# qq456cvb/CanonicalVoting

Measured on AMD Instinct MI355X. Metric: scenes/sec (80k-pt synthetic scans), higher is better.
Workload: dtype f32

## Files before the change

### canonicalvoting_amd/csrc/cv_common.h

```cpp
#pragma once
#include <hip/hip_runtime.h>

#include <cstdarg>
#include <cstdint>
#include <cstdio>

#include "cv_hip.h"

void cv_set_error(const char* fmt, ...);

#define CV_HIP_CHECK(expr)                                                                  \
    do {                                                                                    \
        hipError_t e_ = (expr);                                                             \
        if (e_ != hipSuccess) {                                                             \
            cv_set_error("%s failed: %s (%s:%d)", #expr, hipGetErrorString(e_), __FILE__,   \
                         __LINE__);                                                         \
            return CV_EHIP;                                                                 \
        }                                                                                   \
    } while (0)

#define CV_LAUNCH_CHECK() CV_HIP_CHECK(hipGetLastError())

#define CV_REQUIRE(cond, code, ...)     \
    do {                                \
        if (!(cond)) {                  \
            cv_set_error(__VA_ARGS__);  \
            return (code);              \
        }                               \
    } while (0)

__host__ __device__ static inline size_t cv_align_up(size_t v, size_t a) { return (v + a - 1) / a * a; }

struct CvCarver {
    char* base;
    size_t off = 0;
    explicit CvCarver(void* p) : base(static_cast<char*>(p)) {}
    template <typename T>
    T* take(size_t count) {
        off = cv_align_up(off, 256);
        T* r = reinterpret_cast<T*>(base + off);
        off += count * sizeof(T);
        return r;
    }
};

struct CvMapJob {
    const int32_t* out_coords; long long n_out;
    const unsigned long long* keys; const int32_t* vals; long long cap;
    int k, ts;
    int32_t* nbr;
    const int32_t* compose;
    const unsigned* bitmap;
    const int32_t* bbox;
    int up;
};
constexpr int CV_MAX_MAP_JOBS = 12;
int cv_sp_kernel_maps_batch(const CvMapJob* jobs, int n_jobs, void* stream);
constexpr long long CV_BITMAP_WORDS = 1ll << 20;
int cv_sp_occupancy_bitmap(const int32_t* d_coords, long long n, const int32_t* d_bbox, unsigned* d_bits, void* stream,
                           bool pre_cleared = false);

int cv_sp_build_levels_zero(int32_t* const* d_coords, unsigned long long* const* d_keys, int32_t* const* d_vals,
                            long long n, long long cap, int num_levels, int32_t* d_counts, int32_t* h_counts, void* d_ws,
                            size_t ws_bytes, int32_t* d_zero, long long n_zero, int32_t* d_set_one, void* stream,
                            uint32_t* d_bits = nullptr);

struct CvUpJob { const int32_t* nbr_down; long long n_coarse; int32_t* up; };
int cv_sp_up_maps_batch(const CvUpJob* jobs, int n_jobs, void* stream);

struct CvPermJob { const int32_t* nbr; long long n; int K, groups; int32_t* perm; int with_map; };
constexpr int CV_MAX_PERM_JOBS = 8;
int cv_hv_minmax_async_ex(const float* d_points, int64_t n, float* h_minmax6, void* d_ws, size_t ws_bytes, int32_t* d_zero_word,
                          int32_t* d_fill7f, void* stream);
int cv_decode_f32_ev(float* d_grid_obj, const float* d_grid_rot, const float* d_grid_scale, const int dims[3],
                     const float h_corner3[3], float res, const float* d_points, const float* d_xyz, const float* d_prob,
                     const int32_t* d_class, int64_t n, const cv_decode_params* params, int mutate_grid, void* d_ws, size_t ws_bytes,
                     int* h_n_cand, int64_t* h_cand_idx, int32_t* h_verdict, int* h_n_boxes, float* h_boxes, float* h_scores,
                     int32_t* h_classes, int* h_truncated, void* stream, void* ev_done);
int cv_decode_cat_f32_ev(float* d_grid_obj, const float* d_grid_rot, const float* d_grid_scale, const int dims[3],
                         const float h_corner3[3], float res, const float* d_points, const float* d_xyz, const float* d_prob,
                         const int32_t* d_class, int64_t n, int num_cats, const cv_decode_params* params, int mutate_grid,
                         void* d_ws, size_t ws_bytes, int* h_n_cand, int64_t* h_cand_idx, int32_t* h_verdict, int* h_n_boxes,
                         float* h_boxes, float* h_scores, int32_t* h_classes, int* h_truncated, void* stream, void* ev_done);
int cv_sp_sort_rows_ex(const int32_t* d_coords, long long n, int32_t* d_sorted, int32_t* d_perm, int32_t* d_inv, void* d_ws,
                       size_t ws_bytes, bool single_batch, void* stream, bool bounds_prefilled = false);
int cv_sp_scene_plan_ex(const int32_t* d_input, long long n, int32_t* d_perm, int32_t* d_inv, int32_t* const* d_coords,
                        unsigned long long* const* d_keys, int32_t* const* d_vals, long long cap, int32_t* d_counts,
                        int32_t* h_counts, int stem_k, int mask_groups, long long masked_min_rows,
                        int32_t* d_arena, size_t arena_words, cv_scene_maps* offsets, void* d_sort_ws, size_t sort_ws_bytes,
                        void* d_levels_ws, size_t levels_ws_bytes, bool single_batch, void* stream,
                        bool bounds_prefilled = false);
int cv_sp_mask_perms_batch(const CvPermJob* jobs, int n_jobs, void* d_ws, size_t ws_bytes, void* stream,
                           bool pre_zeroed = false);
```

### canonicalvoting_amd/csrc/net_exec.cpp

```cpp
#include <algorithm>
#include <cstdlib>
#include <mutex>
#include <unordered_map>
#include <vector>

#include "cv_common.h"

namespace {

struct Slot { char* ptr; int ld; long long rows; };

}

extern "C" {

static void scene_maps_layout(const long long* rows, long long n_orig, int stem_k, int mask_groups,
                              long long masked_min_rows, cv_scene_maps* o, size_t* total) {
    size_t off = 0;
    auto take = [&](size_t words) { const size_t at = off; off += cv_align_up(words, 64); return (long long)at; };
    const size_t K5 = (size_t)stem_k * stem_k * stem_k;
    const size_t mp_w = mask_groups > 1 ? (size_t)mask_groups * (1 + (27 + mask_groups - 1) / mask_groups) + (mask_groups + 3) / 4 : 0;
    o->stem = take((size_t)rows[0] * K5);
    o->k3[0] = take((size_t)rows[0] * 27);
    o->mask_perm[0] = (mask_groups > 1 && rows[0] >= masked_min_rows) ? take(mp_w * rows[0]) : -1;
    o->scratch = take((size_t)(5 * std::max(mask_groups, 1) + 4) * 2048);
    o->bitmap = take((size_t)CV_BITMAP_WORDS);
    o->out = -1;
    (void)n_orig;
    for (int i = 0; i < 4; ++i) o->down[i] = take((size_t)rows[i + 1] * 8);
    for (int i = 1; i < 5; ++i) o->k3[i] = take((size_t)rows[i] * 27);
    for (int i = 0; i < 4; ++i) o->up[i] = take((size_t)rows[3 - i] * 8);
    for (int i = 1; i < 5; ++i) o->mask_perm[i] = (mask_groups > 1 && rows[i] >= masked_min_rows) ? take(mp_w * rows[i]) : -1;
    for (int i = 0; i < 4; ++i) o->up_perm[i] = take((size_t)rows[3 - i]);
    *total = off;
}

size_t cv_sp_scene_maps_words(const long long* level_rows, long long n_orig, int stem_k, int mask_groups,
                              long long masked_min_rows, cv_scene_maps* offsets) {
    if (!level_rows || !offsets || n_orig <= 0 || stem_k < 1) return 0;
    size_t total = 0;
    scene_maps_layout(level_rows, n_orig, stem_k, mask_groups, masked_min_rows, offsets, &total);
    return total;
}

static int scene_maps_level0(int32_t* const* d_coords, const unsigned long long* const* d_keys, const int32_t* const* d_vals,
                             long long cap, long long n, const int32_t* d_perm, int stem_k, int mask_groups,
                             const cv_scene_maps& o, int32_t* d_arena, const int32_t* d_bbox, void* stream,
                             bool pre_cleared = false, bool bitmap_filled = false) {
    const unsigned* bits = nullptr;
    if (d_bbox) {
        bits = reinterpret_cast<const unsigned*>(d_arena + o.bitmap);
        if (!bitmap_filled) {
            const int rc0 = cv_sp_occupancy_bitmap(d_coords[0], n, d_bbox, reinterpret_cast<unsigned*>(d_arena + o.bitmap), stream,
                                                   pre_cleared);
            if (rc0 != CV_OK) return rc0;
        }
    }
    CvMapJob mj[2];
    mj[0] = {d_coords[0], n, d_keys[0], d_vals[0], cap, stem_k, 1, d_arena + o.stem, d_perm, bits, d_bbox, 0};
    mj[1] = {d_coords[0], n, d_keys[0], d_vals[0], cap, 3, 1, d_arena + o.k3[0], nullptr, bits, d_bbox, 0};
    int rc = cv_sp_kernel_maps_batch(mj, 2, stream);
    if (rc != CV_OK) return rc;
    if (o.mask_perm[0] >= 0) {
        CvPermJob pj = {d_arena + o.k3[0], n, 27, mask_groups, d_arena + o.mask_perm[0], 1};
        rc = cv_sp_mask_perms_batch(&pj, 1, d_arena + o.scratch, sizeof(int) * (size_t)mask_groups * 2048, stream, pre_cleared);
        if (rc != CV_OK) return rc;
    }
    return CV_OK;
}

static int scene_maps_coarse(int32_t* const* d_coords, const unsigned long long* const* d_keys, const int32_t* const* d_vals,
                             long long cap, const long long* level_rows, int mask_groups, const cv_scene_maps& o,
                             int32_t* d_arena, void* stream, bool pre_zeroed = false) {
    CvMapJob mj[CV_MAX_MAP_JOBS];
    int nm = 0;
    for (int i = 0; i < 4; ++i)
        mj[nm++] = {d_coords[i + 1], level_rows[i + 1], d_keys[i], d_vals[i], cap, 2, 1 << i, d_arena + o.down[i], nullptr, nullptr, nullptr, 0};
    for (int i = 1; i < 5; ++i)
        mj[nm++] = {d_coords[i], level_rows[i], d_keys[i], d_vals[i], cap, 3, 1 << i, d_arena + o.k3[i], nullptr, nullptr, nullptr, 0};
    for (int i = 0; i < 4; ++i) {
        const int fine = 3 - i;
        mj[nm++] = {d_coords[fine], level_rows[fine], d_keys[fine + 1], d_vals[fine + 1], cap, 2, 1 << fine, d_arena + o.up[i],
                    nullptr, nullptr, nullptr, 1};
    }
    int rc = cv_sp_kernel_maps_batch(mj, nm, stream);
    if (rc != CV_OK) return rc;
    CvPermJob pj[CV_MAX_PERM_JOBS];
    int np = 0, groups = 0;
    for (int i = 1; i < 5; ++i)
        if (o.mask_perm[i] >= 0) {
            pj[np++] = {d_arena + o.k3[i], level_rows[i], 27, mask_groups, d_arena + o.mask_perm[i], 1};
            groups += mask_groups;
        }
    for (int i = 0; i < 4; ++i) {
        pj[np++] = {d_arena + o.up[i], level_rows[3 - i], 8, 1, d_arena + o.up_perm[i], 0};
        groups += 1;
    }
    return cv_sp_mask_perms_batch(pj, np, d_arena + o.scratch + (size_t)std::max(mask_groups, 1) * 2048,
                                  sizeof(int) * (size_t)groups * 2048, stream, pre_zeroed);
}

int cv_sp_scene_maps(int32_t* const* d_coords, const unsigned long long* const* d_keys, const int32_t* const* d_vals,
                     long long cap, const long long* level_rows, const int32_t* d_perm, long long n_orig, int stem_k,
                     int mask_groups, long long masked_min_rows, int32_t* d_arena, size_t arena_words, void* stream) {
    CV_REQUIRE(d_coords && d_keys && d_vals && level_rows && d_perm && d_arena, CV_EINVAL, "null pointer argument");
    CV_REQUIRE(n_orig == level_rows[0], CV_EINVAL, "the sorted set must hold the caller's %lld rows", n_orig);
    cv_scene_maps o;
    size_t total = 0;
    scene_maps_layout(level_rows, n_orig, stem_k, mask_groups, masked_min_rows, &o, &total);
    CV_REQUIRE(arena_words >= total, CV_ENOMEM, "scene map arena too small");
    int rc = scene_maps_level0(d_coords, d_keys, d_vals, cap, n_orig, d_perm, stem_k, mask_groups, o, d_arena, nullptr, stream);
    if (rc != CV_OK) return rc;
    return scene_maps_coarse(d_coords, d_keys, d_vals, cap, level_rows, mask_groups, o, d_arena, stream);
}

namespace {
struct PlanSide { hipEvent_t ev; int32_t* h_pinned; int device; };
std::mutex g_plan_mu;
std::unordered_map<int, std::vector<PlanSide>> g_plan_free;
int plan_side_acquire(PlanSide* out) {
    int dev = 0;
    CV_HIP_CHECK(hipGetDevice(&dev));
    {
        std::lock_guard<std::mutex> lk(g_plan_mu);
        auto& pool = g_plan_free[dev];
        if (!pool.empty()) {
            *out = pool.back();
            pool.pop_back();
// ... 178 lines not shown
```

### canonicalvoting_amd/csrc/sparse_conv.hip

```cpp
#include "cv_common.h"

#include <atomic>
#include <cstring>
#include <type_traits>
#include <utility>

#include "sparse_conv_common.h"

using namespace cvsc;

namespace {

template <int NB, bool VEC>
__global__ __launch_bounds__(THREADS) void conv_rows(ConvArgs a) {
    __shared__ float A_s[KC][A_LD];
    __shared__ float B_s[KC][NB * 32];
    __shared__ int nbr_s[TM];
    __shared__ int rows_s[TM];
    __shared__ __attribute__((aligned(16))) float ep_s[4][32][EP_LD];
    const int tid = threadIdx.x, lane = tid & 63, wave = tid >> 6;
    const int n0 = blockIdx.y * (NB * 32);

    if (tid < TM) {
        const long long tile_id = a.row_perm ? (long long)gridDim.x - 1 - blockIdx.x : blockIdx.x;
// ... 1414 lines not shown
        conv_finish_small<<<(unsigned)std::min<long long>((total / 4 + 255) / 256, 16384), 256, 0, st>>>(a);
    else if (a.cout % 4 == 0)
        conv_finish<<<(unsigned)std::min<long long>((total / 4 + 63) / 64, 8192), 256, 0, st>>>(a);
    else
        conv_finish_scalar<<<(unsigned)std::min<long long>((total + 255) / 256, 4096), 256, 0, st>>>(a);
    CV_LAUNCH_CHECK();
    return CV_OK;
}
}
namespace {

__global__ __launch_bounds__(256) void mask_keys(const int* __restrict__ nbr, long long n, int K, int j_begin,
                                                 int j_end, long long* __restrict__ keys) {
    const long long i = blockIdx.x * 256ll + threadIdx.x;
    if (i >= n) return;
    unsigned long long m = 0;
    for (int j = j_begin; j < j_end; ++j)
        if (nbr[i * K + j] >= 0) m |= 1ull << (j - j_begin);
    keys[i] = (long long)m;
}

constexpr int MP_BINS = 1024;
constexpr int MP_THREADS = 1024;

__device__ __forceinline__ int group_mask(const int* __restrict__ nbr, long long row, long long n, int K, int jb, int je) {
    int m = 0;
    for (int j = jb; j < je; ++j)
        if (nbr[row * K + j] >= 0) m |= 1 << (j - jb);
    if (je - jb <= 7) m |= __popc(m) << 7;
    (void)n;
    return m;
}

__global__ __launch_bounds__(MP_THREADS) void mp_hist(const int* __restrict__ nbr, long long n, int K, int groups,
                                                      int* __restrict__ hist ) {
    __shared__ int lh[MP_BINS];
    const int g = blockIdx.y;
    const int jb = K * g / groups, je = K * (g + 1) / groups;
    for (int i = threadIdx.x; i < MP_BINS; i += MP_THREADS) lh[i] = 0;
    __syncthreads();
    const long long row = blockIdx.x * (long long)MP_THREADS + threadIdx.x;
    if (row < n) atomicAdd(&lh[group_mask(nbr, row, n, K, jb, je)], 1);
    __syncthreads();
    for (int i = threadIdx.x; i < MP_BINS; i += MP_THREADS)
        if (lh[i]) atomicAdd(&hist[g * MP_BINS + i], lh[i]);
}

__global__ __launch_bounds__(MP_BINS) void mp_scan(int* __restrict__ hist) {
    __shared__ int s[MP_BINS];
    int* h = hist + blockIdx.x * MP_BINS;
    const int v = h[threadIdx.x];
    s[threadIdx.x] = v;
    __syncthreads();
    for (int off = 1; off < MP_BINS; off <<= 1) {
        const int t = threadIdx.x >= off ? s[threadIdx.x - off] : 0;
        __syncthreads();
        s[threadIdx.x] += t;
        __syncthreads();
    }
    h[threadIdx.x] = s[threadIdx.x] - v;
}

__global__ __launch_bounds__(MP_THREADS) void mp_scatter(const int* __restrict__ nbr, long long n, int K, int groups,
                                                         int* __restrict__ cursor, int* __restrict__ perm,
                                                         int* __restrict__ nbrp, int W) {
    unsigned char* gv = nbrp ? reinterpret_cast<unsigned char*>(nbrp + (long long)groups * n * W) : nullptr;
// ... 14 lines not shown
    __syncthreads();
    if (row < n) {
        const long long pos = (long long)g * n + lh[key] + rank;
        perm[pos] = (int)row;
        if (nbrp) {
            for (int j = jb; j < je; ++j) nbrp[pos * W + (j - jb)] = nbr[row * K + j];
            gv[(long long)g * n + row] = key != 0;
        }
    }
}

struct PermJobsDev {
    CvPermJob j[CV_MAX_PERM_JOBS];
    int group_begin[CV_MAX_PERM_JOBS + 1];
    int n;
};

__device__ __forceinline__ int perm_job_of(const PermJobsDev& jobs, int gy) {
    int ji = 0;
    while (ji + 1 < jobs.n && gy >= jobs.group_begin[ji + 1]) ++ji;
    return ji;
}

__global__ __launch_bounds__(MP_THREADS) void mp_hist_batch(const PermJobsDev jobs, int* __restrict__ hist) {
    __shared__ int lh[MP_BINS];
    const int ji = perm_job_of(jobs, blockIdx.y);
    const CvPermJob& jb = jobs.j[ji];
    const long long row = blockIdx.x * (long long)MP_THREADS + threadIdx.x;
    if (blockIdx.x * (long long)MP_THREADS >= jb.n) return;
    const int g = blockIdx.y - jobs.group_begin[ji];
    const int jlo = jb.K * g / jb.groups, jhi = jb.K * (g + 1) / jb.groups;
    for (int i = threadIdx.x; i < MP_BINS; i += MP_THREADS) lh[i] = 0;
    __syncthreads();
    if (row < jb.n) atomicAdd(&lh[group_mask(jb.nbr, row, jb.n, jb.K, jlo, jhi)], 1);
    __syncthreads();
    for (int i = threadIdx.x; i < MP_BINS; i += MP_THREADS)
        if (lh[i]) atomicAdd(&hist[blockIdx.y * MP_BINS + i], lh[i]);
}

__global__ __launch_bounds__(MP_THREADS) void mp_scatter_batch(const PermJobsDev jobs, const int* __restrict__ hist,
                                                               int* __restrict__ cursor) {
    static_assert(MP_THREADS == MP_BINS, "one bin per thread in the scan");
    __shared__ int lh[MP_BINS];
    __shared__ int pre[MP_BINS];
    __shared__ int wtot[MP_THREADS / 64];
    const int ji = perm_job_of(jobs, blockIdx.y);
    const CvPermJob& jb = jobs.j[ji];
    if (blockIdx.x * (long long)MP_THREADS >= jb.n) return;
    const int g = blockIdx.y - jobs.group_begin[ji];
    const int K = jb.K, jlo = K * g / jb.groups, jhi = K * (g + 1) / jb.groups, W = (K + jb.groups - 1) / jb.groups;
    int* nbrp = jb.with_map ? jb.perm + (long long)jb.groups * jb.n : nullptr;
    for (int i = threadIdx.x; i < MP_BINS; i += MP_THREADS) lh[i] = 0;
    {
        const int lane = threadIdx.x & 63, wave = threadIdx.x >> 6;
        const int v = hist[blockIdx.y * MP_BINS + threadIdx.x];
        int incl = v;
#pragma unroll
        for (int off = 1; off < 64; off <<= 1) {
            const int t = __shfl_up(incl, off);
            if (lane >= off) incl += t;
        }
        if (lane == 63) wtot[wave] = incl;
        __syncthreads();
        int base = 0;
#pragma unroll
        for (int w = 0; w < MP_THREADS / 64; ++w) base += w < wave ? wtot[w] : 0;
        pre[threadIdx.x] = base + incl - v;
    }
    __syncthreads();
    const long long row = blockIdx.x * (long long)MP_THREADS + threadIdx.x;
    int key = 0, rank = 0;
    if (row < jb.n) {
        key = group_mask(jb.nbr, row, jb.n, K, jlo, jhi);
        rank = atomicAdd(&lh[key], 1);
    }
    __syncthreads();
    for (int i = threadIdx.x; i < MP_BINS; i += MP_THREADS)
        if (lh[i]) lh[i] = pre[i] + atomicAdd(&cursor[blockIdx.y * MP_BINS + i], lh[i]);
    __syncthreads();
    if (row < jb.n) {
        const long long pos = (long long)g * jb.n + lh[key] + rank;
        jb.perm[pos] = (int)row;
        if (nbrp) {
            for (int j = jlo; j < jhi; ++j) nbrp[pos * W + (j - jlo)] = jb.nbr[row * K + j];
            reinterpret_cast<unsigned char*>(nbrp + (long long)jb.groups * jb.n * W)[(long long)g * jb.n + row] = key != 0;
        }
    }
}

__global__ __launch_bounds__(256) void affine_rows(const float* __restrict__ x, long long n, int c,
                                                   int x_ld, const float* __restrict__ scale,
                                                   const float* __restrict__ shift,
                                                   const float* __restrict__ residual, int res_ld, int relu,
                                                   float* __restrict__ y, int y_ld) {
    for (long long t = blockIdx.x * 256ll + threadIdx.x; t < n * c; t += (long long)gridDim.x * 256) {
        const long long r = t / c;
        const int k = (int)(t - r * c);
        float v = x[r * x_ld + k];
        if (scale) v = v * scale[k] + (shift ? shift[k] : 0.f);
        if (residual) v += residual[r * res_ld + k];
        if (relu) v = fmaxf(v, 0.f);
        y[r * y_ld + k] = v;
    }
}

__global__ __launch_bounds__(256) void affine_rows4(const float* __restrict__ x, long long n, int c,
                                                    int x_ld, const float* __restrict__ scale,
                                                    const float* __restrict__ shift,
                                                    const float* __restrict__ residual, int res_ld, int relu,
                                                    float* __restrict__ y, int y_ld, float* __restrict__ y_hl = nullptr,
                                                    int y_hl_ld = 0, int* __restrict__ range_flag = nullptr,
                                                    unsigned* __restrict__ ybits = nullptr) {
    const int cq = c >> 2;
    for (long long t = blockIdx.x * 256ll + threadIdx.x; t < n * cq; t += (long long)gridDim.x * 256) {
        const long long r = t / cq;
        const int k = (int)(t - r * cq) * 4;
        float4 v = *reinterpret_cast<const float4*>(x + r * x_ld + k);
        if (scale) {
            const float4 sc = *reinterpret_cast<const float4*>(scale + k);
// ... 484 lines not shown
    CV_REQUIRE(name && value, CV_EINVAL, "null option name / value");
    const std::atomic<long long>* o = !strcmp(name, "hd_mask") ? &g_opt_hd_mask : !strcmp(name, "hd_min_rows") ? &g_opt_hd_min_rows :
                                      !strcmp(name, "hd_shape") ? &g_opt_hd_shape : !strcmp(name, "zskip") ? &g_opt_zskip : nullptr;
    CV_REQUIRE(o, CV_EINVAL, "unknown option '%s'", name);
    *value = o->load(std::memory_order_relaxed);
    return CV_OK;
}

int cv_sp_set_ablation(int bits) { return cvsc::g_ablation.exchange(bits, std::memory_order_relaxed); }

int cv_sp_set_split_target_thread(int workgroups) {
    const int before = (int)t_split_target;
    t_split_target = workgroups > 0 ? workgroups : 0;
    return before;
}

int cv_sp_set_split_target(int workgroups) {
    const int before = (int)process_split_target();
    g_split_target.store(workgroups > 0 ? workgroups : -1, std::memory_order_relaxed);
    return before;
}

int cv_sp_mask_perms_batch(const CvPermJob* jobs, int n_jobs, void* d_ws, size_t ws_bytes, void* stream, bool pre_zeroed) {
    CV_REQUIRE(jobs && d_ws && n_jobs > 0 && n_jobs <= CV_MAX_PERM_JOBS, CV_EINVAL, "bad mask perm batch");
    PermJobsDev d;
    d.n = n_jobs;
    int groups = 0;
    long long max_n = 0;
    for (int i = 0; i < n_jobs; ++i) {
        const CvPermJob& j = jobs[i];
        CV_REQUIRE(j.nbr && j.perm && j.n > 0 && j.K > 0 && j.groups >= 1 && j.groups <= j.K, CV_EINVAL,
                   "bad mask perm job %d", i);
        CV_REQUIRE((j.K + j.groups - 1) / j.groups <= 10, CV_EINVAL, "at most 10 kernel offsets per group");
        d.j[i] = j;
        d.group_begin[i] = groups;
        groups += j.groups;
        max_n = std::max(max_n, j.n);
    }
    d.group_begin[n_jobs] = groups;
    CV_REQUIRE(ws_bytes >= sizeof(int) * (size_t)groups * MP_BINS * 2, CV_ENOMEM, "workspace too small");
    hipStream_t st = static_cast<hipStream_t>(stream);
    int* hist = static_cast<int*>(d_ws);
    int* cursor = hist + (size_t)groups * MP_BINS;
    if (!pre_zeroed) CV_HIP_CHECK(hipMemsetAsync(hist, 0, sizeof(int) * (size_t)groups * MP_BINS * 2, st));
    dim3 grid((unsigned)((max_n + MP_THREADS - 1) / MP_THREADS), (unsigned)groups);
    mp_hist_batch<<<grid, MP_THREADS, 0, st>>>(d, hist);
    CV_LAUNCH_CHECK();
    mp_scatter_batch<<<grid, MP_THREADS, 0, st>>>(d, hist, cursor);
    CV_LAUNCH_CHECK();
    return CV_OK;
}

extern "C" {

size_t cv_sp_conv_workspace_bytes(long long n_out, int cout, int K) {
    if (n_out <= 0 || cout <= 0 || K <= 0) return 0;
    const size_t one = sizeof(float) * (size_t)n_out * (size_t)cout;
    return 256 + std::min<size_t>(64 * one, std::max<size_t>((size_t)48 << 20, 3 * one));
}

int cv_sp_conv_f32(const cv_conv_desc* d, void* stream) {
    CV_REQUIRE(d, CV_EINVAL, "null descriptor");
    CV_REQUIRE(d->in && d->weight && d->out, CV_EINVAL, "null pointer argument");
    CV_REQUIRE(d->n_in > 0 && d->n_out > 0 && d->cin > 0 && d->cout > 0 && d->K > 0, CV_EINVAL, "bad conv sizes");
    CV_REQUIRE(d->nbr || (d->K == 1 && d->n_in == d->n_out), CV_EINVAL, "a kernel map is required unless K == 1");
    CV_REQUIRE(d->in_ld >= d->cin && d->out_ld >= d->cout && (!d->residual || d->res_ld >= d->cout) &&
// ... 578 lines not shown
```

### canonicalvoting_amd/csrc/sparse_coords.hip

```cpp
#include "cv_common.h"

#include <limits>

namespace {

constexpr unsigned long long EMPTY_KEY = ~0ull;

__host__ __device__ __forceinline__ unsigned long long pack_key(int b, int x, int y, int z) {
    return ((unsigned long long)(unsigned)(b & 0xffff) << 48) |
           ((unsigned long long)(unsigned)((x + 32768) & 0xffff) << 32) |
           ((unsigned long long)(unsigned)((y + 32768) & 0xffff) << 16) |
           (unsigned long long)(unsigned)((z + 32768) & 0xffff);
}

__device__ __forceinline__ unsigned long long mix64(unsigned long long k) {
    k ^= k >> 33; k *= 0xff51afd7ed558ccdull; k ^= k >> 33; k *= 0xc4ceb9fe1a85ec53ull; k ^= k >> 33;
    return k;
}

__device__ __forceinline__ int floor_div(int a, int b) {
    const int q = a / b;
    return (a % b != 0 && a < 0) ? q - 1 : q;
}

// ... 251 lines not shown
template <int KK>
__device__ __forceinline__ void map_job(const CvMapJob& jb, int nblk, int blk) {
    const int k = KK > 0 ? (KK == 125 ? 5 : KK == 27 ? 3 : 2) : jb.k;
    const int K = KK > 0 ? KK : k * k * k, ts = jb.ts;
    const int lo = (k & 1) ? -(k / 2) : 0;
    const long long mask = jb.cap - 1;
    BitBox bb;
    bb.ok = false;
    if (jb.bitmap && ts == 1) bb = bitbox(jb.bbox);
    const long long total = jb.n_out * K;
    const bool small = total < (1ll << 31);
    for (long long t = blk * 256ll + threadIdx.x; t < total; t += (long long)nblk * 256) {
        long long u;
        int j;
        if (small) { const unsigned tu = (unsigned)t, uu = tu / (unsigned)K; u = uu; j = (int)(tu - uu * (unsigned)K); }
        else { u = t / K; j = (int)(t - u * K); }
        const int ox = lo + j % k, oy = lo + (j / k) % k, oz = lo + j / (k * k);
        const int4 c = reinterpret_cast<const int4*>(jb.out_coords)[u];
        int r = -1;
        bool probe = true;
        if (bb.ok) {
            const long long bit = bitbox_index(bb, c.x, c.y + ox, c.z + oy, c.w + oz);
            probe = bit >= 0 && ((jb.bitmap[bit >> 5] >> (bit & 31)) & 1u);
        }
        if (probe) {
            const long long slot = table_find(jb.keys, mask, pack_key(c.x, c.y + ox * ts, c.z + oy * ts, c.w + oz * ts));
            r = slot >= 0 ? jb.vals[slot] : -1;
            if (jb.compose && r >= 0) r = jb.compose[r];
        }
        jb.nbr[t] = r;
    }
}

__device__ __forceinline__ void up_job(const CvMapJob& jb, int nblk, int blk) {
    const long long mask = jb.cap - 1;
    const int ts = jb.ts, m = ~(2 * ts - 1);
    for (long long f = blk * 256ll + threadIdx.x; f < jb.n_out; f += (long long)nblk * 256) {
        const int4 c = reinterpret_cast<const int4*>(jb.out_coords)[f];
        const int px = c.y & m, py = c.z & m, pz = c.w & m;
        const long long slot = table_find(jb.keys, mask, pack_key(c.x, px, py, pz));
        const int parent = slot >= 0 ? jb.vals[slot] : -1;
        const int oct = ((c.y - px) / ts) + 2 * ((c.z - py) / ts) + 4 * ((c.w - pz) / ts);
        int4 lo = make_int4(-1, -1, -1, -1), hi = lo;
        switch (oct) {
            case 0: lo.x = parent; break; case 1: lo.y = parent; break; case 2: lo.z = parent; break; case 3: lo.w = parent; break;
            case 4: hi.x = parent; break; case 5: hi.y = parent; break; case 6: hi.z = parent; break; default: hi.w = parent; break;
        }
        reinterpret_cast<int4*>(jb.nbr)[2 * f] = lo;
        reinterpret_cast<int4*>(jb.nbr)[2 * f + 1] = hi;
    }
}

__global__ __launch_bounds__(256) void build_kernel_maps(const MapJobsDev jobs) {
    int ji = 0;
    while (ji + 1 < jobs.n && (int)blockIdx.x >= jobs.block_begin[ji + 1]) ++ji;
    const CvMapJob& jb = jobs.j[ji];
    const int nblk = jobs.block_begin[ji + 1] - jobs.block_begin[ji], blk = blockIdx.x - jobs.block_begin[ji];
    if (jb.up) { up_job(jb, nblk, blk); return; }
    switch (jb.k) {
        case 5: map_job<125>(jb, nblk, blk); break;
        case 3: map_job<27>(jb, nblk, blk); break;
        case 2: map_job<8>(jb, nblk, blk); break;
        default: map_job<0>(jb, nblk, blk); break;
    }
}

struct UpJobsDev {
    CvUpJob j[4];
    int block_begin[5];
    int n;
};

__global__ __launch_bounds__(256) void build_up_maps(const UpJobsDev jobs) {
    int ji = 0;
    while (ji + 1 < jobs.n && (int)blockIdx.x >= jobs.block_begin[ji + 1]) ++ji;
    const CvUpJob& jb = jobs.j[ji];
    const int nblk = jobs.block_begin[ji + 1] - jobs.block_begin[ji], blk = blockIdx.x - jobs.block_begin[ji];
    const long long n = jb.n_coarse * 8;
    for (long long t = blk * 256ll + threadIdx.x; t < n; t += (long long)nblk * 256) {
        const int f = jb.nbr_down[t];
        if (f >= 0) jb.up[(long long)f * 8 + (t & 7)] = (int)(t >> 3);
    }
}

__global__ void set_int(int* p, int v) { *p = v; }

__device__ __forceinline__ unsigned long long spread3(unsigned long long v) {
    v &= 0xffffull;
    v = (v | (v << 32)) & 0x00ff00000000ffffull;
    v = (v | (v << 16)) & 0x00ff0000ff0000ffull;
    v = (v | (v << 8)) & 0xf00f00f00f00f00full;
// ... 343 lines not shown
extern "C" {

size_t cv_sp_quantize_workspace_bytes(long long m) {
    if (m <= 0) return 0;
    const size_t cap = (size_t)cv_sp_table_capacity(m);
    return cv_align_up(cap * 8, 256) + cv_align_up(cap * 4, 256) + cv_align_up((size_t)m * 4, 256) + 4096 + 256;
}

int cv_sp_quantize_f32(const float* d_points, long long m, long long ld, float quantization_size, int floor_only,
                       const long long* h_offsets, int n_clouds, int32_t* d_coords4, int32_t* d_index, int32_t* d_inverse,
                       int32_t* d_counts, int32_t* h_counts, void* d_ws, size_t ws_bytes, void* stream) {
    return quantize_run<float>(d_points, m, ld, quantization_size, floor_only, h_offsets, n_clouds, d_coords4, d_index,
                               d_inverse, d_counts, h_counts, d_ws, ws_bytes, stream);
}

int cv_sp_quantize_f64(const double* d_points, long long m, long long ld, double quantization_size, int floor_only,
                       const long long* h_offsets, int n_clouds, int32_t* d_coords4, int32_t* d_index, int32_t* d_inverse,
                       int32_t* d_counts, int32_t* h_counts, void* d_ws, size_t ws_bytes, void* stream) {
    return quantize_run<double>(d_points, m, ld, quantization_size, floor_only, h_offsets, n_clouds, d_coords4, d_index,
                                d_inverse, d_counts, h_counts, d_ws, ws_bytes, stream);
}

}

int cv_sp_kernel_maps_batch(const CvMapJob* jobs, int n_jobs, void* stream) {
    CV_REQUIRE(jobs && n_jobs > 0 && n_jobs <= CV_MAX_MAP_JOBS, CV_EINVAL, "bad kernel map batch");
    MapJobsDev d;
    d.n = n_jobs;
    int total = 0;
    for (int i = 0; i < n_jobs; ++i) {
        const CvMapJob& j = jobs[i];
        CV_REQUIRE(j.out_coords && j.keys && j.vals && j.nbr && j.n_out > 0 && j.k >= 1 && j.k <= 7 && j.ts >= 1,
                   CV_EINVAL, "bad kernel map job %d", i);
        d.j[i] = j;
        d.block_begin[i] = total;
        total += j.up ? grid_for(j.n_out) : grid_for(j.n_out * j.k * j.k * j.k);
    }
    d.block_begin[n_jobs] = total;
    build_kernel_maps<<<total, 256, 0, static_cast<hipStream_t>(stream)>>>(d);
    CV_LAUNCH_CHECK();
    return CV_OK;
}

int cv_sp_occupancy_bitmap(const int32_t* d_coords, long long n, const int32_t* d_bbox, unsigned* d_bits, void* stream,
                           bool pre_cleared) {
    CV_REQUIRE(d_coords && d_bbox && d_bits && n > 0, CV_EINVAL, "bad bitmap arguments");
    hipStream_t st = static_cast<hipStream_t>(stream);
    int* mm = const_cast<int*>(d_bbox);
    if (!pre_cleared) {
        bitmap_clear<<<256, 256, 0, st>>>(d_coords, n, mm, d_bits);
        CV_LAUNCH_CHECK();
    }
    bitmap_set<<<grid_for(n), 256, 0, st>>>(d_coords, n, mm, d_bits);
    CV_LAUNCH_CHECK();
    return CV_OK;
}

int cv_sp_up_maps_batch(const CvUpJob* jobs, int n_jobs, void* stream) {
    CV_REQUIRE(jobs && n_jobs > 0 && n_jobs <= 4, CV_EINVAL, "bad up map batch");
    UpJobsDev d;
    d.n = n_jobs;
    int total = 0;
    for (int i = 0; i < n_jobs; ++i) {
        CV_REQUIRE(jobs[i].nbr_down && jobs[i].up && jobs[i].n_coarse > 0, CV_EINVAL, "bad up map job %d", i);
        d.j[i] = jobs[i];
        d.block_begin[i] = total;
        total += grid_for(jobs[i].n_coarse * 8);
    }
    d.block_begin[n_jobs] = total;
// ... 156 lines not shown
```

Measured before the change: 605.4.

## Fuse stem 5x5x5 and 3x3x3 neighbour maps, emit validity words, coalesce permuted copies

For stem_k = 5, one line-based job now builds both the 5x5x5 and the 3x3x3 kernel maps. It reads a 5-bit z-run of the occupancy bitmap per (x,y) line and probes the hash table for only the occupied cells. The 3x3x3 map jobs write a per-row 27-bit validity word through a wave ballot, and the mask-permutation kernels read that word instead of re-reading 27 neighbour entries. The permuted neighbour copy is restructured into a block-cooperative, coalesced read loop. This adds an extra word per row to the arena and makes the map kernel more complex, and it also adds profiling scripts.

```diff
diff --git a/canonicalvoting_amd/csrc/cv_common.h b/canonicalvoting_amd/csrc/cv_common.h
--- a/canonicalvoting_amd/csrc/cv_common.h
+++ b/canonicalvoting_amd/csrc/cv_common.h
@@ -53,6 +53,8 @@
     const unsigned* bitmap;
     const int32_t* bbox;
     int up;
+    int32_t* nbr3;
+    int32_t* mask_words;
 };
 constexpr int CV_MAX_MAP_JOBS = 12;
 int cv_sp_kernel_maps_batch(const CvMapJob* jobs, int n_jobs, void* stream);
@@ -68,7 +70,10 @@
 struct CvUpJob { const int32_t* nbr_down; long long n_coarse; int32_t* up; };
 int cv_sp_up_maps_batch(const CvUpJob* jobs, int n_jobs, void* stream);
 
-struct CvPermJob { const int32_t* nbr; long long n; int K, groups; int32_t* perm; int with_map; };
+struct CvPermJob {
+    const int32_t* nbr; long long n; int K, groups; int32_t* perm; int with_map;
+    const int32_t* mask_words;
+};
 constexpr int CV_MAX_PERM_JOBS = 8;
 int cv_hv_minmax_async_ex(const float* d_points, int64_t n, float* h_minmax6, void* d_ws, size_t ws_bytes, int32_t* d_zero_word,
                           int32_t* d_fill7f, void* stream);
diff --git a/canonicalvoting_amd/csrc/net_exec.cpp b/canonicalvoting_amd/csrc/net_exec.cpp
--- a/canonicalvoting_amd/csrc/net_exec.cpp
+++ b/canonicalvoting_amd/csrc/net_exec.cpp
@@ -21,18 +21,22 @@
     const size_t K5 = (size_t)stem_k * stem_k * stem_k;
     const size_t mp_w = mask_groups > 1 ? (size_t)mask_groups * (1 + (27 + mask_groups - 1) / mask_groups) + (mask_groups + 3) / 4 : 0;
     o->stem = take((size_t)rows[0] * K5);
-    o->k3[0] = take((size_t)rows[0] * 27);
+    o->k3[0] = take((size_t)rows[0] * 28);
     o->mask_perm[0] = (mask_groups > 1 && rows[0] >= masked_min_rows) ? take(mp_w * rows[0]) : -1;
     o->scratch = take((size_t)(5 * std::max(mask_groups, 1) + 4) * 2048);
     o->bitmap = take((size_t)CV_BITMAP_WORDS);
     o->out = -1;
     (void)n_orig;
     for (int i = 0; i < 4; ++i) o->down[i] = take((size_t)rows[i + 1] * 8);
-    for (int i = 1; i < 5; ++i) o->k3[i] = take((size_t)rows[i] * 27);
+    for (int i = 1; i < 5; ++i) o->k3[i] = take((size_t)rows[i] * 28);
     for (int i = 0; i < 4; ++i) o->up[i] = take((size_t)rows[3 - i] * 8);
     for (int i = 1; i < 5; ++i) o->mask_perm[i] = (mask_groups > 1 && rows[i] >= masked_min_rows) ? take(mp_w * rows[i]) : -1;
     for (int i = 0; i < 4; ++i) o->up_perm[i] = take((size_t)rows[3 - i]);
     *total = off;
+}
+
+static int32_t* scene_mask_words(int32_t* d_arena, const cv_scene_maps& o, int level, long long rows) {
+    return d_arena + o.k3[level] + rows * 27;
 }
 
 size_t cv_sp_scene_maps_words(const long long* level_rows, long long n_orig, int stem_k, int mask_groups,
@@ -57,12 +61,19 @@
         }
     }
     CvMapJob mj[2];
-    mj[0] = {d_coords[0], n, d_keys[0], d_vals[0], cap, stem_k, 1, d_arena + o.stem, d_perm, bits, d_bbox, 0};
-    mj[1] = {d_coords[0], n, d_keys[0], d_vals[0], cap, 3, 1, d_arena + o.k3[0], nullptr, bits, d_bbox, 0};
-    int rc = cv_sp_kernel_maps_batch(mj, 2, stream);
+    int32_t* mw = scene_mask_words(d_arena, o, 0, n);
+    int nm = 1;
+    if (stem_k == 5) {
+        mj[0] = {d_coords[0], n, d_keys[0], d_vals[0], cap, 5, 1, d_arena + o.stem, d_perm, bits, d_bbox, 0, d_arena + o.k3[0], mw};
+    } else {
+        mj[0] = {d_coords[0], n, d_keys[0], d_vals[0], cap, stem_k, 1, d_arena + o.stem, d_perm, bits, d_bbox, 0, nullptr, nullptr};
+        mj[1] = {d_coords[0], n, d_keys[0], d_vals[0], cap, 3, 1, d_arena + o.k3[0], nullptr, bits, d_bbox, 0, nullptr, mw};
+        nm = 2;
+    }
+    int rc = cv_sp_kernel_maps_batch(mj, nm, stream);
     if (rc != CV_OK) return rc;
     if (o.mask_perm[0] >= 0) {
-        CvPermJob pj = {d_arena + o.k3[0], n, 27, mask_groups, d_arena + o.mask_perm[0], 1};
+        CvPermJob pj = {d_arena + o.k3[0], n, 27, mask_groups, d_arena + o.mask_perm[0], 1, mw};
         rc = cv_sp_mask_perms_batch(&pj, 1, d_arena + o.scratch, sizeof(int) * (size_t)mask_groups * 2048, stream, pre_cleared);
         if (rc != CV_OK) return rc;
     }
@@ -75,13 +86,15 @@
     CvMapJob mj[CV_MAX_MAP_JOBS];
     int nm = 0;
     for (int i = 0; i < 4; ++i)
-        mj[nm++] = {d_coords[i + 1], level_rows[i + 1], d_keys[i], d_vals[i], cap, 2, 1 << i, d_arena + o.down[i], nullptr, nullptr, nullptr, 0};
+        mj[nm++] = {d_coords[i + 1], level_rows[i + 1], d_keys[i], d_vals[i], cap, 2, 1 << i, d_arena + o.down[i], nullptr, nullptr, nullptr, 0,
+                    nullptr, nullptr};
     for (int i = 1; i < 5; ++i)
-        mj[nm++] = {d_coords[i], level_rows[i], d_keys[i], d_vals[i], cap, 3, 1 << i, d_arena + o.k3[i], nullptr, nullptr, nullptr, 0};
+        mj[nm++] = {d_coords[i], level_rows[i], d_keys[i], d_vals[i], cap, 3, 1 << i, d_arena + o.k3[i], nullptr, nullptr, nullptr, 0,
+                    nullptr, o.mask_perm[i] >= 0 ? scene_mask_words(d_arena, o, i, level_rows[i]) : nullptr};
     for (int i = 0; i < 4; ++i) {
         const int fine = 3 - i;
         mj[nm++] = {d_coords[fine], level_rows[fine], d_keys[fine + 1], d_vals[fine + 1], cap, 2, 1 << fine, d_arena + o.up[i],
-                    nullptr, nullptr, nullptr, 1};
+                    nullptr, nullptr, nullptr, 1, nullptr, nullptr};
     }
     int rc = cv_sp_kernel_maps_batch(mj, nm, stream);
     if (rc != CV_OK) return rc;
@@ -89,11 +102,12 @@
     int np = 0, groups = 0;
     for (int i = 1; i < 5; ++i)
         if (o.mask_perm[i] >= 0) {
-            pj[np++] = {d_arena + o.k3[i], level_rows[i], 27, mask_groups, d_arena + o.mask_perm[i], 1};
+            pj[np++] = {d_arena + o.k3[i], level_rows[i], 27, mask_groups, d_arena + o.mask_perm[i], 1,
+                        scene_mask_words(d_arena, o, i, level_rows[i])};
             groups += mask_groups;
         }
     for (int i = 0; i < 4; ++i) {
-        pj[np++] = {d_arena + o.up[i], level_rows[3 - i], 8, 1, d_arena + o.up_perm[i], 0};
+        pj[np++] = {d_arena + o.up[i], level_rows[3 - i], 8, 1, d_arena + o.up_perm[i], 0, nullptr};
         groups += 1;
     }
     return cv_sp_mask_perms_batch(pj, np, d_arena + o.scratch + (size_t)std::max(mask_groups, 1) * 2048,
diff --git a/canonicalvoting_amd/csrc/sparse_conv.hip b/canonicalvoting_amd/csrc/sparse_conv.hip
--- a/canonicalvoting_amd/csrc/sparse_conv.hip
+++ b/canonicalvoting_amd/csrc/sparse_conv.hip
@@ -1470,6 +1470,12 @@
     return m;
 }
 
+__device__ __forceinline__ int group_mask_of_word(int word, int jb, int je) {
+    int m = (int)(((unsigned)word >> jb) & ((1u << (je - jb)) - 1u));
+    if (je - jb <= 7) m |= __popc(m) << 7;
+    return m;
+}
+
 __global__ __launch_bounds__(MP_THREADS) void mp_hist(const int* __restrict__ nbr, long long n, int K, int groups,
                                                       int* __restrict__ hist ) {
     __shared__ int lh[MP_BINS];
@@ -1550,7 +1556,8 @@
     const int jlo = jb.K * g / jb.groups, jhi = jb.K * (g + 1) / jb.groups;
     for (int i = threadIdx.x; i < MP_BINS; i += MP_THREADS) lh[i] = 0;
     __syncthreads();
-    if (row < jb.n) atomicAdd(&lh[group_mask(jb.nbr, row, jb.n, jb.K, jlo, jhi)], 1);
+    if (row < jb.n)
+        atomicAdd(&lh[jb.mask_words ? group_mask_of_word(jb.mask_words[row], jlo, jhi) : group_mask(jb.nbr, row, jb.n, jb.K, jlo, jhi)], 1);
     __syncthreads();
     for (int i = threadIdx.x; i < MP_BINS; i += MP_THREADS)
         if (lh[i]) atomicAdd(&hist[blockIdx.y * MP_BINS + i], lh[i]);
@@ -1589,20 +1596,39 @@
     const long long row = blockIdx.x * (long long)MP_THREADS + threadIdx.x;
     int key = 0, rank = 0;
     if (row < jb.n) {
-        key = group_mask(jb.nbr, row, jb.n, K, jlo, jhi);
+        key = jb.mask_words ? group_mask_of_word(jb.mask_words[row], jlo, jhi) : group_mask(jb.nbr, row, jb.n, K, jlo, jhi);
         rank = atomicAdd(&lh[key], 1);
     }
     __syncthreads();
     for (int i = threadIdx.x; i < MP_BINS; i += MP_THREADS)
         if (lh[i]) lh[i] = pre[i] + atomicAdd(&cursor[blockIdx.y * MP_BINS + i], lh[i]);
     __syncthreads();
+    long long pos = 0;
     if (row < jb.n) {
-        const long long pos = (long long)g * jb.n + lh[key] + rank;
+        pos = (long long)g * jb.n + lh[key] + rank;
         jb.perm[pos] = (int)row;
-        if (nbrp) {
-            for (int j = jlo; j < jhi; ++j) nbrp[pos * W + (j - jlo)] = jb.nbr[row * K + j];
-            reinterpret_cast<unsigned char*>(nbrp + (long long)jb.groups * jb.n * W)[(long long)g * jb.n + row] = key != 0;
-        }
+        if (nbrp) reinterpret_cast<unsigned char*>(nbrp + (long long)jb.groups * jb.n * W)[(long long)g * jb.n + row] = key != 0;
+    }
+    if (!nbrp) return;
+    pre[threadIdx.x] = (int)(pos - (long long)g * jb.n);
+    __syncthreads();
+    const long long row0 = blockIdx.x * (long long)MP_THREADS;
+    const int nrow = (int)((jb.n - row0 < MP_THREADS) ? jb.n - row0 : MP_THREADS), Wg = jhi - jlo;
+    const int total = nrow * Wg;
+    const int* src0 = jb.nbr + row0 * K + jlo;
+    int* dst0 = nbrp + (long long)g * jb.n * W;
+    for (int e0 = threadIdx.x; e0 < total; e0 += 3 * MP_THREADS) {
+        int v[3], r[3], jj[3];
+#pragma unroll
+        for (int q = 0; q < 3; ++q) {
+            const int e = e0 + q * MP_THREADS;
+            r[q] = Wg == 9 ? (int)((unsigned)e / 9u) : (int)((unsigned)e / (unsigned)Wg);
+            jj[q] = e - r[q] * Wg;
+            v[q] = e < total ? src0[(long long)r[q] * K + jj[q]] : 0;
+        }
+#pragma unroll
+        for (int q = 0; q < 3; ++q)
+            if (e0 + q * MP_THREADS < total) dst0[(long long)pre[r[q]] * W + jj[q]] = v[q];
     }
 }
 
@@ -2153,6 +2179,7 @@
         CV_REQUIRE(j.nbr && j.perm && j.n > 0 && j.K > 0 && j.groups >= 1 && j.groups <= j.K, CV_EINVAL,
                    "bad mask perm job %d", i);
         CV_REQUIRE((j.K + j.groups - 1) / j.groups <= 10, CV_EINVAL, "at most 10 kernel offsets per group");
+        CV_REQUIRE(!j.mask_words || j.K <= 32, CV_EINVAL, "validity words hold at most 32 kernel offsets");
         d.j[i] = j;
         d.group_begin[i] = groups;
         groups += j.groups;
diff --git a/canonicalvoting_amd/csrc/sparse_coords.hip b/canonicalvoting_amd/csrc/sparse_coords.hip
--- a/canonicalvoting_amd/csrc/sparse_coords.hip
+++ b/canonicalvoting_amd/csrc/sparse_coords.hip
@@ -307,6 +307,123 @@
     }
 }
 
+__device__ __forceinline__ void map_rows27(const CvMapJob& jb, int* __restrict__ nbr, const int* __restrict__ compose, int nblk,
+                                           int blk) {
+    const int ts = jb.ts;
+    const long long mask = jb.cap - 1;
+    BitBox bb;
+    bb.ok = false;
+    if (jb.bitmap && ts == 1) bb = bitbox(jb.bbox);
+    const int lane = threadIdx.x & 63, hl = lane & 31;
+    const int ox = hl % 3 - 1, oy = (hl / 3) % 3 - 1, oz = hl / 9 - 1;
+    for (long long u0 = blk * 8ll; u0 < jb.n_out; u0 += nblk * 8ll) {
+        const long long u = u0 + (threadIdx.x >> 5);
+        const bool act = u < jb.n_out && hl < 27;
+        int r = -1;
+        if (act) {
+            const int4 c = reinterpret_cast<const int4*>(jb.out_coords)[u];
+            bool probe = true;
+            if (bb.ok) {
+                const long long bit = bitbox_index(bb, c.x, c.y + ox, c.z + oy, c.w + oz);
+                probe = bit >= 0 && ((jb.bitmap[bit >> 5] >> (bit & 31)) & 1u);
+            }
+            if (probe) {
+                const long long slot = table_find(jb.keys, mask, pack_key(c.x, c.y + ox * ts, c.z + oy * ts, c.w + oz * ts));
+                r = slot >= 0 ? jb.vals[slot] : -1;
+                if (compose && r >= 0) r = compose[r];
+            }
+            nbr[u * 27 + hl] = r;
+        }
+        const unsigned long long b = __ballot(r >= 0);
+        if (act && hl == 0 && jb.mask_words) jb.mask_words[u] = (int)((unsigned)(b >> (lane & 32)) & 0x7ffffffu);
+    }
+}
+
+__device__ __forceinline__ void line_job(const CvMapJob& jb, int nblk, int blk) {
+    BitBox bb;
+    bb.ok = false;
+    if (jb.bitmap) bb = bitbox(jb.bbox);
+    if (!bb.ok) {
+        map_job<125>(jb, nblk, blk);
+        map_rows27(jb, jb.nbr3, nullptr, nblk, blk);
+        return;
+    }
+    const long long mask = jb.cap - 1;
+    const int lane = threadIdx.x & 63, hl = lane & 31;
+    const bool line = hl < 25;
+    const int dx = hl % 5 - 2, dy = hl / 5 - 2;
+    const bool inner = line && dx >= -1 && dx <= 1 && dy >= -1 && dy <= 1;
+    const int line3 = (dx + 1) + 3 * (dy + 1);
+    for (long long u0 = blk * 8ll; u0 < jb.n_out; u0 += nblk * 8ll) {
+        const long long u = u0 + (threadIdx.x >> 5);
+        const bool have = u < jb.n_out && line;
+        int4 c = make_int4(0, 0, 0, 0);
+        unsigned m5 = 0;
+        if (have) {
+            c = reinterpret_cast<const int4*>(jb.out_coords)[u];
+            const int ux = c.y + dx - bb.mn[0], uy = c.z + dy - bb.mn[1], uz = c.w - bb.mn[2];
+            const int zlo = max(uz - 2, 0), zhi = min(uz + 2, bb.d[2] - 1);
+            if ((unsigned)ux < (unsigned)bb.d[0] && (unsigned)uy < (unsigned)bb.d[1] && (unsigned)c.x < (unsigned)bb.nb &&
+                zlo <= zhi) {
+                const long long first = (((long long)c.x * bb.d[0] + ux) * bb.d[1] + uy) * bb.d[2] + zlo;
+                const int sh = (int)(first & 31), nbits = zhi - zlo + 1;
+                unsigned long long v = jb.bitmap[first >> 5];
+                if (sh + nbits > 32) v |= (unsigned long long)jb.bitmap[(first >> 5) + 1] << 32;
+                m5 = ((unsigned)(v >> sh) & ((1u << nbits) - 1u)) << (zlo - (uz - 2));
+            }
+        }
+        unsigned long long key[5], kk[5];
+        long long sl[5];
+#pragma unroll
+        for (int k = 0; k < 5; ++k) {
+            key[k] = pack_key(c.x, c.y + dx, c.z + dy, c.w + k - 2);
+            sl[k] = ((m5 >> k) & 1u) ? (long long)(mix64(key[k]) & (unsigned long long)mask) : 0;
+        }
+#pragma unroll
+        for (int k = 0; k < 5; ++k) kk[k] = jb.keys[sl[k]];
+#pragma unroll
+        for (int k = 0; k < 5; ++k)
+            if ((m5 >> k) & 1u)
+                while (kk[k] != key[k] && kk[k] != EMPTY_KEY) {
+                    sl[k] = (sl[k] + 1) & mask;
+                    kk[k] = jb.keys[sl[k]];
+                }
+        int r[5], rc[5];
+        bool hit[5];
+#pragma unroll
+        for (int k = 0; k < 5; ++k) {
+            hit[k] = ((m5 >> k) & 1u) && kk[k] == key[k];
+            r[k] = jb.vals[hit[k] ? sl[k] : 0];
+        }
+#pragma unroll
+        for (int k = 0; k < 5; ++k) {
+            r[k] = hit[k] ? r[k] : -1;
+            rc[k] = r[k];
+        }
+        if (jb.compose) {
+#pragma unroll
+            for (int k = 0; k < 5; ++k) rc[k] = jb.compose[r[k] >= 0 ? r[k] : 0];
+#pragma unroll
+            for (int k = 0; k < 5; ++k) rc[k] = r[k] >= 0 ? rc[k] : -1;
+        }
+        if (have) {
+#pragma unroll
+            for (int k = 0; k < 5; ++k) jb.nbr[u * 125 + k * 25 + hl] = rc[k];
+        }
+        if (have && inner) {
+#pragma unroll
+            for (int k = 1; k < 4; ++k) jb.nbr3[u * 27 + (k - 1) * 9 + line3] = r[k];
+        }
+        unsigned w = 0;
+#pragma unroll
+        for (int k = 1; k < 4; ++k) {
+            const unsigned h = (unsigned)(__ballot(have && inner && r[k] >= 0) >> (lane & 32));
+            w |= (((h >> 6) & 7u) | (((h >> 11) & 7u) << 3) | (((h >> 16) & 7u) << 6)) << ((k - 1) * 9);
+        }
+        if (have && hl == 0 && jb.mask_words) jb.mask_words[u] = (int)w;
+    }
+}
+
 __device__ __forceinline__ void up_job(const CvMapJob& jb, int nblk, int blk) {
     const long long mask = jb.cap - 1;
     const int ts = jb.ts, m = ~(2 * ts - 1);
@@ -332,6 +449,8 @@
     const CvMapJob& jb = jobs.j[ji];
     const int nblk = jobs.block_begin[ji + 1] - jobs.block_begin[ji], blk = blockIdx.x - jobs.block_begin[ji];
     if (jb.up) { up_job(jb, nblk, blk); return; }
+    if (jb.nbr3) { line_job(jb, nblk, blk); return; }
+    if (jb.mask_words) { map_rows27(jb, jb.nbr, jb.compose, nblk, blk); return; }
     switch (jb.k) {
         case 5: map_job<125>(jb, nblk, blk); break;
         case 3: map_job<27>(jb, nblk, blk); break;
@@ -741,9 +860,12 @@
         const CvMapJob& j = jobs[i];
         CV_REQUIRE(j.out_coords && j.keys && j.vals && j.nbr && j.n_out > 0 && j.k >= 1 && j.k <= 7 && j.ts >= 1,
                    CV_EINVAL, "bad kernel map job %d", i);
+        CV_REQUIRE(!j.nbr3 || (j.k == 5 && j.ts == 1 && !j.up), CV_EINVAL, "job %d: the combined 5x5x5 + 3x3x3 map is a ts = 1 map", i);
+        CV_REQUIRE(!j.mask_words || j.nbr3 || (j.k == 3 && !j.up), CV_EINVAL, "job %d: validity words belong to a 3x3x3 map", i);
         d.j[i] = j;
         d.block_begin[i] = total;
-        total += j.up ? grid_for(j.n_out) : grid_for(j.n_out * j.k * j.k * j.k);
+        total += j.up ? grid_for(j.n_out) : (j.nbr3 || j.mask_words) ? (int)std::min<long long>((j.n_out + 7) / 8, 16384)
+                                                                       : grid_for(j.n_out * j.k * j.k * j.k);
     }
     d.block_begin[n_jobs] = total;
     build_kernel_maps<<<total, 256, 0, static_cast<hipStream_t>(stream)>>>(d);
diff --git a/profiles/plan_launches.py b/profiles/plan_launches.py
--- /dev/null
+++ b/profiles/plan_launches.py
@@ -0,0 +1,58 @@
+import collections
+import csv
+import gzip
+import json
+import statistics
+import sys
+
+from in_flight_summary import family, find
+
+
+def main():
+    tdir, bench_json = sys.argv[1:3]
+    label = sys.argv[3] if len(sys.argv) > 3 else ""
+    bench = json.loads(open(bench_json).read().strip().splitlines()[-1])
+    steps = bench["steps"]
+    tfile = tdir if tdir.endswith((".gz", ".csv")) else find(tdir, "kernel_trace.csv")
+    rows = list(csv.DictReader(gzip.open(tfile, "rt") if tfile.endswith(".gz") else open(tfile)))
+
+    def grid(r):
+        g = [int(r[k]) for k in ("Grid_Size_X", "Grid_Size_Y", "Grid_Size_Z")]
+        w = [max(1, int(r[k])) for k in ("Workgroup_Size_X", "Workgroup_Size_Y", "Workgroup_Size_Z")]
+        return g[0] // w[0], max(1, g[1] // w[1])
+
+    ev = sorted((int(r["Start_Timestamp"]), int(r["End_Timestamp"]), r["Kernel_Name"], grid(r)) for r in rows)
+    heads = [e for e in ev if family(e[2]) == "head"]
+    iso = 2 * 4 + max(min(steps, 48), 24)
+    assert len(heads) >= steps + iso, (len(heads), steps, iso)
+    t_lo, t_hi = heads[-(steps + iso) + 20][0], heads[-(iso + 20) - 1][1]
+    t_iso = heads[-(iso - 8) - 1][1]
+    dur = {"in flight": collections.defaultdict(list), "alone": collections.defaultdict(list)}
+    for s, e, n, g in ev:
+        if family(n) != "plan":
+            continue
+        short = n.replace("(anonymous namespace)::", "").replace("void ", "").split("(")[0]
+        where = "in flight" if t_lo < s < t_hi else "alone" if s > t_iso else None
+        if where:
+            dur[where][(short, g)].append((e - s) * 1e-3)
+    scenes = {"in flight": len([h for h in heads if t_lo < h[1] <= t_hi]), "alone": iso - 8}
+    print("%s: plan launches, median us (launches per scene) - %.1f scenes/s under the tracer" % (label, bench["value"]))
+    print("%-26s %6s %3s %18s %18s" % ("kernel", "wgs", "y", "in flight", "alone"))
+    keys = sorted(set(dur["in flight"]) | set(dur["alone"]), key=lambda k: (k[0], -k[1][0], k[1][1]))
+    tot = {"in flight": 0.0, "alone": 0.0}
+    for k in keys:
+        cells = []
+        for w in ("in flight", "alone"):
+            v = dur[w].get(k)
+            if v:
+                per = len(v) / scenes[w]
+                tot[w] += sum(v) / scenes[w]
+                cells.append("%8.1f (%4.2f)" % (statistics.median(v), per))
+            else:
+                cells.append("%15s" % "-")
+        print("%-26s %6d %3d %18s %18s" % (k[0][:26], k[1][0], k[1][1], cells[0], cells[1]))
+    print("%-26s %10s %18.1f %18.1f   (sum of plan kernel time per scene, us)" % ("all plan launches", "", tot["in flight"], tot["alone"]))
+
+
+if __name__ == "__main__":
+    main()
diff --git a/profiles/supertile_pricing.py b/profiles/supertile_pricing.py
--- /dev/null
+++ b/profiles/supertile_pricing.py
@@ -0,0 +1,92 @@
+import os
+import sys
+
+import numpy as np
+
+sys.path.insert(0, os.path.dirname(os.path.dirname(os.path.abspath(__file__))))
+from canonicalvoting_amd.synth import make_scene
+
+SIZES = (256, 512, 1024, 2048, 4096, 8192, 16384, None)
+
+
+def spread3(x):
+    r = np.zeros_like(x)
+    for b in range(6):
+        r |= ((x >> b) & 1) << (3 * b)
+    return r
+
+
+def plan_order(c):
+    mn = c.min(0)
+    ex = int((c.max(0) - mn).max())
+    shift = 0
+    while (ex >> shift) >= 64:
+        shift += 1
+    g = (c - mn) >> shift
+    key = spread3(g[:, 0]) | (spread3(g[:, 1]) << 1) | (spread3(g[:, 2]) << 2)
+    return c[np.argsort(key, kind="stable")]
+
+
+def coarser(c, ts):
+    q = c & ~(2 * ts - 1)
+    _, first = np.unique(pack(q), return_index=True)
+    return q[np.sort(first)]
+
+
+def pack(c):
+    return ((c[:, 0] + 32768) << 40) | ((c[:, 1] + 32768) << 20) | (c[:, 2] + 32768)
+
+
+def live_table(c, ts):
+    keys = pack(c)
+    order = np.argsort(keys)
+    sk = keys[order]
+    live = np.zeros((len(c), 27), bool)
+    j = 0
+    for dz in (-1, 0, 1):
+        for dy in (-1, 0, 1):
+            for dx in (-1, 0, 1):
+                q = pack(c + np.array([dx, dy, dz]) * ts)
+                pos = np.minimum(np.searchsorted(sk, q), len(sk) - 1)
+                live[:, j] = sk[pos] == q
+                j += 1
+    return live
+
+
+def units(live, S):
+    n = len(live)
+    tile = np.arange(n) // S if S else np.zeros(n, np.int64)
+    nblk = (n + 31) // 32
+    pad = nblk * 32 - n
+    tot = 0
+    for g in range(3):
+        lv = live[:, 9 * g:9 * g + 9]
+        mask = (lv * (1 << np.arange(9))).sum(1)
+        o = np.lexsort((mask, tile))
+        l2 = np.concatenate([lv[o], np.zeros((pad, 9), bool)])
+        tot += int(l2.reshape(nblk, 32, 9).any(1).sum())
+    return tot / (27.0 * nblk)
+
+
+def main():
+    sc = make_scene(0, n_points=80000, res=0.03)
+    c = plan_order(np.asarray(sc.coords, np.int64))
+    levels = [("ts1", c, 1)]
+    c2 = coarser(c, 1)
+    levels.append(("ts2", c2, 2))
+    levels.append(("ts4", coarser(c2, 2), 4))
+    print("live (32-row block, offset) units / (27 per block); three groups of nine offsets; sort key (row // S, group mask)")
+    print("%-14s " % "S rows" + " ".join("%7s" % (s if s else "inf") for s in SIZES))
+    res = {}
+    for name, cc, ts in levels:
+        live = live_table(cc, ts)
+        res[name] = [units(live, s) for s in SIZES]
+        print("%-14s " % ("%s (%d)" % (name, len(cc))) + " ".join("%7.3f" % u for u in res[name]))
+    fit = SIZES.index(4096)
+    print("\nts1: the partial sums (S x 96 x 4 B) and input rows of a super-tile fit a 4 MB XCD L2 for S <= 4096: %.2f x today's units"
+          % (res["ts1"][fit] / res["ts1"][-1]))
+    print("(pairs live: " + ", ".join("%s %.1f %%" % (n_, 100 * live_table(c_, t_).mean()) for n_, c_, t_ in levels) + ")")
+
+
+if __name__ == "__main__":
+    main()
```

Measured after the change: 629.5 (median of 6 runs). 1.04x the previous value.
